# paroj/aruco

Measured on AMD Instinct MI355X. Metric: frames/sec at 1920×1080, higher is better.
Workload: dtype u8

## Files before the change

aruco_amd/capi.py:

```python
import ctypes as C
import os
import sys

import numpy as np

from .build import library_path

OK, E_INVALID, E_CAPACITY, E_UNSUPPORTED, E_HIP, E_OVERFLOW, E_BOARD_CONFIG = range(7)
THRES_FIXED, THRES_ADPT, THRES_CANNY = 0, 1, 2
CORNER_NONE, CORNER_HARRIS, CORNER_SUBPIX, CORNER_LINES = 0, 1, 2, 3
BOARD_NONE, BOARD_PIX, BOARD_METERS = -1, 0, 1

_ERR_NAMES = {1: "ARUCOHIP_E_INVALID", 2: "ARUCOHIP_E_CAPACITY", 3: "ARUCOHIP_E_UNSUPPORTED", 4: "ARUCOHIP_E_HIP",
              5: "ARUCOHIP_E_OVERFLOW", 6: "ARUCOHIP_E_BOARD_CONFIG"}


class ArucoHipError(RuntimeError):
    def __init__(self, code, msg=""):
        super().__init__("%s (%d): %s" % (_ERR_NAMES.get(code, "error"), code, msg))
        self.code = code


class Params(C.Structure):
    _fields_ = [("thres_method", C.c_int32), ("thres_param1_range", C.c_int32), ("thres_param1", C.c_double),
# ... 23 lines not shown
assert MARKER_DTYPE.itemsize == 96 and C.sizeof(Marker) == 96

SYMBOLS = [
    "arucohip_version", "arucohip_default_params", "arucohip_default_limits", "arucohip_create", "arucohip_create_ex",
    "arucohip_destroy", "arucohip_set_params", "arucohip_get_params", "arucohip_last_error_string", "arucohip_set_stream",
    "arucohip_get_stream", "arucohip_synchronize", "arucohip_detect", "arucohip_detect_batch", "arucohip_batch_status", "arucohip_batch_chunks",
    "arucohip_get_thresholded", "arucohip_get_candidates", "arucohip_threshold", "arucohip_detect_rectangles",
    "arucohip_warp", "arucohip_debug_num_contours", "arucohip_debug_contour", "arucohip_debug_candidates", "arucohip_debug_otsu",
    "arucohip_board_detect", "arucohip_calculate_extrinsics", "arucohip_stage_times", "arucohip_stage_name",
    "arucohip_enable_timing", "arucohip_kernel_times", "arucohip_threshold_exec_ms", "arucohip_kernel_name",
    "arucohip_debug_counters", "arucohip_board_detect_batch",
    "arucohip_gl_modelview", "arucohip_ogre_pose", "arucohip_gl_projection", "arucohip_ogre_projection",
    "arucohip_detect_bgr", "arucohip_detect_batch_bgr", "arucohip_bgr_to_gray", "arucohip_set_dictionary",
    "arucohip_set_decoder_callback",
    "arucohip_undistort", "arucohip_gl_modelview_n", "arucohip_gl_modelview_batch",
    "arucohip_set_pipeline_depth", "arucohip_detect_batch_submit", "arucohip_detect_batch_wait",
    "arucohip_mgpu_device_count", "arucohip_mgpu_create", "arucohip_mgpu_destroy", "arucohip_mgpu_size", "arucohip_mgpu_handle",
    "arucohip_mgpu_set_params", "arucohip_mgpu_last_error_string", "arucohip_mgpu_detect_batch", "arucohip_mgpu_detect_streams",
    "arucohip_mgpu_set_depth", "arucohip_mgpu_submit_batch", "arucohip_mgpu_submit_streams", "arucohip_mgpu_wait",
    "arucohip_compact_bytes", "arucohip_compact_markers", "arucohip_wait_event", "arucohip_detect_batch_retry_overflowed",
    "arucohip_refine_candidate_lines", "arucohip_mgpu_gather_mode", "arucohip_build_info",
]

_lib = None


def load():
    global _lib
    if _lib is not None:
        return _lib
    path = os.environ.get("ARUCOHIP_LIB") or library_path()
# ... 306 lines not shown

    def submit_host(self, frames, out, n, K=None, dist=None, marker_size=-1.0, y_perp=False):
        nf, h, w = frames.shape
        Ka, da = _f32(K), _f32(dist)
        t = C.c_int(-1)
        self._chk(self.L.arucohip_detect_batch_submit(self.h, _ptr(frames), nf, w, h, w, w * h, 0, _ptr(Ka), _ptr(da), 0 if da is None else da.size,
                                                      float(marker_size), int(bool(y_perp)), _ptr(out), out.shape[1], _ptr(n), 0, C.byref(t)))
        return t.value

    def wait(self, ticket, allow=()):
        return self._chk(self.L.arucohip_detect_batch_wait(self.h, int(ticket)), allow)

    def batch_status(self):
        return self._chk(self.L.arucohip_batch_status(self.h))

    def batch_chunks(self):
        per = C.c_int(0)
        n = self.L.arucohip_batch_chunks(self.h, C.byref(per))
        return n, per.value

    def thresholded(self, frame=0, shape=None):
        out = np.empty(shape, np.uint8)
        self._chk(self.L.arucohip_get_thresholded(self.h, frame, _ptr(out)))
        return out

    def candidates(self, frame=0, cap=512):
        q = np.zeros((cap, 4, 2), np.float32)
        n = C.c_int(0)
        self._chk(self.L.arucohip_get_candidates(self.h, frame, _ptr(q), cap, C.byref(n)))
        return q[:n.value].copy()
# ... 224 lines not shown
```

aruco_amd/csrc/capi.hip:

```cpp
#include <hip/hip_runtime.h>

#include <algorithm>
#include <cmath>
#include <cstdio>
#include <cstring>
#include <string>
#include <vector>

#include "bits_tiles.h"
#include "internal.h"

namespace ah {
void launch_rotate_x(hipStream_t s, double* rt);
}

namespace ah {
Tuning read_tuning() {
    Tuning t;
    auto geti = [](const char* name, int dflt) {
        const char* e = getenv(name);
        return (e && *e) ? atoi(e) : dflt;
    };
    t.walk_fork = geti("ARUCOHIP_WALK_FORK", 1) != 0;
    t.chain = geti("ARUCOHIP_CHAIN", 0) != 0;
    t.cand_sparse = geti("ARUCOHIP_CAND_SPARSE", 1) != 0;
    t.cand_waves = std::max(1, geti("ARUCOHIP_CAND_WAVES", 32));
    t.cand_chunks = std::max(1, geti("ARUCOHIP_CAND_CHUNKS", 16));
    t.leash = geti("ARUCOHIP_LEASH", 0);
    t.fork_after = geti("ARUCOHIP_FORK_AFTER", 3);
    t.quad_blocks = std::max(1, geti("ARUCOHIP_QUAD_BLOCKS", 12));
    t.quad_dual = geti("ARUCOHIP_QUAD_DUAL", 1) != 0;
    t.seg_skip = geti("ARUCOHIP_SEG_SKIP", 1) != 0;
    t.gen_xcd = geti("ARUCOHIP_GEN_XCD", 1) != 0;
    t.threshold_wide = geti("ARUCOHIP_THRESHOLD_WIDE", 1) != 0;
    t.threshold_eo = geti("ARUCOHIP_THRESHOLD_EO", 1) != 0;
#ifdef ARUCOHIP_STAGE_EXPERIMENT
    t.stop_after = geti("ARUCOHIP_STOP_AFTER", 99);
#endif
    t.thres_lazy = geti("ARUCOHIP_THRES_BYTES", 0) == 0;
// ... 41 lines not shown
            p = nullptr;
        return e;
    }

private:
    hipError_t release() {
        const hipError_t e = p ? (pinned ? hipHostFree(p) : hipFree(p)) : hipSuccess;
        p = nullptr, bytes = 0;
        return e;
    }
};

struct arucohip_handle {
    int device = 0;
    hipStream_t own_stream = nullptr, stream = nullptr;
    arucohip_params_t params;
    arucohip_limits_t lim;
    Buffers buf{};
    uint64_t alloc_epoch = 0;
    std::vector<Mem<void>> held;
    Mem<uint32_t> walk_scratch;
    Mem<uint8_t> patches;
    Mem<uint8_t> d_gray;
    Mem<uint8_t> d_bgr;
    arucohip_marker_t* wt_out = nullptr;
    int32_t* wt_n = nullptr;
    int wt_cap = 0;
    Mem<uint8_t> d_erode;
    Mem<uint64_t> d_canny;
    Mem<short2> d_umap_xy;
// ... 41 lines not shown
    int last_chunks = 1, last_per = 0;
    struct FrameGraph {
        hipGraphExec_t exec = nullptr;
        uint64_t key = 0;
        uint64_t seen = 0;
        uint64_t epoch = 0;
        bool thres_bytes = false;
        int disabled = 0;
    } fgraph;
    std::vector<arucohip_handle*> lanes;
    int next_ticket = 0;
    arucohip_handle* cur = nullptr;
    arucohip_handle* retry = nullptr;
    int retry_mult = 0;
    hipEvent_t ev_submit = nullptr;
    struct Pending {
        bool active = false;
        int ticket = -1, nframes = 0, cap = 0, out_on_device = 0;
        arucohip_marker_t* out = nullptr;
        int32_t* n_out = nullptr;
    } pend;
    std::string err;
};

static arucohip_handle* active(arucohip_handle* h) { return (h && h->cur) ? h->cur : h; }

static arucohip_handle* route(arucohip_handle* h, int frame, int* local) {
    if (h->last_chunks <= 1 || h->last_per <= 0) {
        *local = frame;
        return h;
    }
    const int c = std::min(frame / h->last_per, h->last_chunks - 1);
    *local = frame - c * h->last_per;
    return c == 0 ? h : h->kids[c - 1];
}

#define HIPCHK(h, expr)                                                                         \
    do {                                                                                        \
        hipError_t e_ = (expr);                                                                 \
        if (e_ != hipSuccess) {                                                                 \
// ... 63 lines not shown
    if (p->use_locked_corners && (p->corner_method == ARUCOHIP_CORNER_HARRIS || p->corner_method == ARUCOHIP_CORNER_SUBPIX) &&
        ((int)p->thres_param1 < 1 || (int)p->thres_param1 > 31))
        return fail(h, ARUCOHIP_E_UNSUPPORTED, "locked corners: window (thres_param1) outside 1..31");
    if (p->decoder_kind < ARUCOHIP_DECODER_FIDUCIAL_5X5 || p->decoder_kind > ARUCOHIP_DECODER_USER) return fail(h, ARUCOHIP_E_INVALID, "bad decoder kind");
    if (p->thres_param1_range < 0 || 2 * p->thres_param1_range + 1 > 16) return fail(h, ARUCOHIP_E_UNSUPPORTED, "threshold range too large");
    if (p->corner_method == ARUCOHIP_CORNER_SUBPIX && (int)p->thres_param1 > 15) return fail(h, ARUCOHIP_E_UNSUPPORTED, "SUBPIX window > 15");
    if (p->corner_method == ARUCOHIP_CORNER_SUBPIX && (int)p->thres_param1 < 1) return fail(h, ARUCOHIP_E_INVALID, "SUBPIX window < 1");
    return ARUCOHIP_OK;
}

extern "C" void arucohip_destroy(arucohip_handle* h);
static void free_all(arucohip_handle* h) {
    hipSetDevice(h->device);
    for (auto* k : h->kids) arucohip_destroy(k);
    h->kids.clear();
    for (auto* l : h->lanes) arucohip_destroy(l);
    h->lanes.clear();
    if (h->retry) arucohip_destroy(h->retry);
    h->retry = nullptr;
    if (h->fgraph.exec) hipGraphExecDestroy(h->fgraph.exec);
    h->fgraph.exec = nullptr;
    if (h->ev_submit) hipEventDestroy(h->ev_submit);
    if (h->ev_fork) hipEventDestroy(h->ev_fork);
    if (h->ev_thr) hipEventDestroy(h->ev_thr);
    if (h->ev_wfork) hipEventDestroy(h->ev_wfork);
    if (h->ev_wjoin) hipEventDestroy(h->ev_wjoin);
    if (h->side_stream) hipStreamDestroy(h->side_stream);
    for (auto& e : h->ev_join)
        if (e) hipEventDestroy(e);
    for (auto& set : h->ev)
        for (auto& e : set)
            if (e) hipEventDestroy(e);
    if (h->own_stream) hipStreamDestroy(h->own_stream);
}

static thread_local bool g_creating_child = false;

static void drop_retry(arucohip_handle* h) {
    if (h->retry) arucohip_destroy(h->retry);
    h->retry = nullptr, h->retry_mult = 0;
}

int arucohip_create_ex(const arucohip_params_t* params, int device, const arucohip_limits_t* lim, arucohip_handle** out) {
    if (!out || !lim) return ARUCOHIP_E_INVALID;
    *out = nullptr;
    if (lim->max_width < 32 || lim->max_height < 32 || lim->max_width > 16383 || lim->max_height > 16383 || lim->max_batch < 1 ||
        lim->max_thres_planes < 1 || lim->max_thres_planes > 16 || lim->candidates_per_frame > 512 || lim->markers_per_frame > 256 ||
        (long)lim->max_width * lim->max_height > (1L << 26) )
        return ARUCOHIP_E_INVALID;
    arucohip_handle* h = new arucohip_handle();
    h->device = device;
// ... 3 lines not shown
    else
        arucohip_default_params(&h->params);
    int rc = validate_params(h, &h->params);
    if (rc != ARUCOHIP_OK) {
        delete h;
        return rc;
    }
    auto bail = [&](hipError_t e) {
        fprintf(stderr, "arucohip_create: %s\n", hipGetErrorString(e));
        free_all(h);
        delete h;
        return ARUCOHIP_E_HIP;
    };
    hipError_t e;
    if ((e = hipSetDevice(device)) != hipSuccess) return bail(e);
    if ((e = hipStreamCreateWithFlags(&h->own_stream, hipStreamNonBlocking)) != hipSuccess) return bail(e);
    h->stream = h->own_stream;
    {
        const double mpx = (double)lim->max_batch * lim->max_width * lim->max_height / (128.0 * 1024 * 1024);
        int ns = 1;
        (void)mpx;
        if (const char* es = getenv("ARUCOHIP_STREAMS")) ns = std::min(8, std::max(1, atoi(es)));
        if (g_creating_child) ns = 1;
        h->is_child = g_creating_child;
        h->nsub = std::min(ns, lim->max_batch);
        h->cap_frames = (lim->max_batch + h->nsub - 1) / h->nsub;
    }
    const size_t F = h->cap_frames, P = F * lim->max_thres_planes, px = (size_t)lim->max_width * lim->max_height;
    Buffers& b = h->buf;
    b.tune = read_tuning();
    {
        const char* eg = getenv("ARUCOHIP_GRAPH");
// ... 66 lines not shown
        b.raw_cnt = b.trig_cnt + w_plane;
        b.ring_cnt = b.raw_cnt + w_plane;
    }
    ALLOC(h->d_small_f, 8192 * sizeof(float));
    ALLOC(h->d_small_d, 64 * sizeof(double));
    ALLOC(h->d_small_i, 64 * sizeof(int));
    ALLOC(h->d_patch, 128 * 128);
#undef ALLOC
    if ((e = hold(h, h->h_markers, (F * b.cap_markers + 1) * sizeof(arucohip_marker_t), true)) != hipSuccess) return bail(e);
    if ((e = hold(h, h->h_n, F * sizeof(int32_t), true)) != hipSuccess) return bail(e);
    if ((e = hold(h, h->h_counters, (CNT_FIXED + F) * sizeof(uint32_t), true)) != hipSuccess) return bail(e);
    for (auto& set : h->ev)
        for (auto& ev : set)
            if ((e = hipEventCreate(&ev)) != hipSuccess) return bail(e);
    if ((e = hipEventCreateWithFlags(&h->ev_thr, hipEventDisableTiming)) != hipSuccess) return bail(e);
    if ((e = hipStreamCreateWithFlags(&h->side_stream, hipStreamNonBlocking)) != hipSuccess) return bail(e);
    if ((e = hipEventCreateWithFlags(&h->ev_wfork, hipEventDisableTiming)) != hipSuccess) return bail(e);
    if ((e = hipEventCreateWithFlags(&h->ev_wjoin, hipEventDisableTiming)) != hipSuccess) return bail(e);
    if (h->nsub > 1) {
        if ((e = hipEventCreateWithFlags(&h->ev_fork, hipEventDisableTiming)) != hipSuccess) return bail(e);
        for (int i = 0; i < h->nsub - 1; i++) {
            if ((e = hipEventCreateWithFlags(&h->ev_join[i], hipEventDisableTiming)) != hipSuccess) return bail(e);
            arucohip_limits_t kl = *lim;
            kl.max_batch = h->cap_frames;
            arucohip_handle* kid = nullptr;
            g_creating_child = true;
            int krc = arucohip_create_ex(&h->params, device, &kl, &kid);
            g_creating_child = false;
            if (krc != ARUCOHIP_OK) {
                free_all(h);
                delete h;
// ... 52 lines not shown

int arucohip_synchronize(arucohip_handle* h) {
    if (!h) return ARUCOHIP_E_INVALID;
    HIPCHK(h, hipSetDevice(h->device));
    HIPCHK(h, hipStreamSynchronize(h->stream));
    return ARUCOHIP_OK;
}

int arucohip_wait_event(arucohip_handle* h, void* ev) {
    if (!h || !ev) return ARUCOHIP_E_INVALID;
    HIPCHK(h, hipSetDevice(h->device));
    HIPCHK(h, hipStreamWaitEvent(h->stream, (hipEvent_t)ev, 0));
    return ARUCOHIP_OK;
}

int arucohip_enable_timing(arucohip_handle* h, int on) {
    if (!h) return ARUCOHIP_E_INVALID;
    h->timing = on == 1;
    h->tsets = 0;
    for (auto* k : h->kids) k->timing = h->timing, k->tsets = 0;
    auto arm = [&](arucohip_handle* x) {
        x->buf.thr_stamp_on = on != 0 && x->buf.thr_stamps && x->buf.thr_acc;
        if (on && x->buf.thr_acc) {
            hipSetDevice(x->device);
            (void)hipStreamSynchronize(x->stream);
            (void)hipMemset(x->buf.thr_acc, 0, 2 * sizeof(uint64_t));
        }
    };
    arm(h);
    for (auto* k : h->kids) arm(k);
    for (auto* l : h->lanes) arucohip_enable_timing(l, on);
    return ARUCOHIP_OK;
}
static void collect_times(arucohip_handle* h) {
    for (int k = 0; k < K_COUNT; k++) h->kernel_ms[k] = 0;
    hipSetDevice(h->device);
    int total = 0;
    auto add = [&](arucohip_handle* w) {
        int n = std::min(w->tsets, TSETS);
        if (n <= 0) return;
        if (hipStreamSynchronize(w->stream) != hipSuccess) return;
        for (int s = 0; s < n; s++)
            for (int k = 0; k < K_COUNT; k++) {
                float ms = 0;
                if (hipEventElapsedTime(&ms, w->ev[s][k], w->ev[s][k + 1]) == hipSuccess) h->kernel_ms[k] += ms;
            }
        total += n;
    };
    add(h);
    for (auto* k : h->kids) add(k);
    for (auto* l : h->lanes) {
        add(l);
        for (auto* k : l->kids) add(k);
    }
    if (total > 0)
        for (int k = 0; k < K_COUNT; k++) h->kernel_ms[k] /= total;
// ... 5 lines not shown
    for (int i = 0; i < STAGE_COUNT && i < cap; i++) ms[i] = 0;
    for (int k = 0; k < K_COUNT; k++)
        if (kKernelStage[k] < cap) ms[kKernelStage[k]] += h->kernel_ms[k];
    return STAGE_COUNT;
}
const char* arucohip_kernel_name(int i) { return (i >= 0 && i < K_COUNT) ? kKernelNames[i] : ""; }
int arucohip_threshold_exec_ms(arucohip_handle* h, double* total_ms, int* launches) {
    if (!h || !total_ms || !launches) return ARUCOHIP_E_INVALID;
    hipSetDevice(h->device);
    int khz = 0;
    if (hipDeviceGetAttribute(&khz, hipDeviceAttributeWallClockRate, h->device) != hipSuccess || khz <= 0) return fail(h, ARUCOHIP_E_HIP, "no wall clock rate");
    unsigned long long ticks = 0, n = 0;
    auto add = [&](arucohip_handle* w) -> int {
        if (!w->buf.thr_acc) return ARUCOHIP_OK;
        unsigned long long v[2] = {0, 0};
        HIPCHK(h, hipStreamSynchronize(w->stream));
        HIPCHK(h, hipMemcpy(v, w->buf.thr_acc, sizeof(v), hipMemcpyDeviceToHost));
        ticks += v[0], n += v[1];
        return ARUCOHIP_OK;
    };
    int rc = add(h);
    for (auto* k : h->kids) if (rc == ARUCOHIP_OK) rc = add(k);
    for (auto* l : h->lanes) {
        if (rc == ARUCOHIP_OK) rc = add(l);
        for (auto* k : l->kids) if (rc == ARUCOHIP_OK) rc = add(k);
    }
    if (rc != ARUCOHIP_OK) return rc;
    *total_ms = (double)ticks / (double)khz, *launches = (int)n;
    return ARUCOHIP_OK;
}

// ... 86 lines not shown
    if (need > 0xFFFFFFF0ull) return fail(h, ARUCOHIP_E_CAPACITY, "batch too large for 32-bit checkpoint offsets: fewer frames per batch or a smaller max size");
    HIPCHK(h, h->walk_scratch.reserve(need * sizeof(uint32_t), h->alloc_epoch));
    h->buf.walk_scratch = h->walk_scratch;
    return ARUCOHIP_OK;
}

static int batch_prologue(arucohip_handle* h, const FrameGeom& g, int nframes, const DetectParams& dp) {
    int rc;
    if ((rc = ensure_walk_scratch(h, nframes * dp.nthr, dp))) return rc;
    if ((rc = ensure_bits_geometry(h, g.width, g.height))) return rc;
    HIPCHK(h, h->patches.reserve((size_t)h->buf.cap_flat * dp.warp_size * dp.warp_size, h->alloc_epoch));
    h->buf.patches = h->patches;
    return ARUCOHIP_OK;
}

static int user_decode_stage(arucohip_handle* h, const DetectParams& dp) {
    hipStream_t s = h->stream;
    const Buffers& b = h->buf;
    const size_t npx = (size_t)dp.warp_size * dp.warp_size;
    HIPCHK(h, h->hu_list.reserve((size_t)b.cap_flat * (sizeof(uint32_t) + sizeof(int2) + sizeof(uint32_t)) + sizeof(uint32_t), h->alloc_epoch));
    uint32_t* list = h->hu_list;
    int2* dec = (int2*)(list + b.cap_flat);
    uint32_t* order = (uint32_t*)(dec + b.cap_flat);
    uint32_t* ncand_p = order + b.cap_flat;
    HIPCHK(h, hipMemcpyAsync(ncand_p, b.counters + CNT_NCAND, sizeof(uint32_t), hipMemcpyDeviceToHost, s));
    HIPCHK(h, hipStreamSynchronize(s));
    const uint32_t n = std::min(*ncand_p, b.cap_flat);
    if (!n) return ARUCOHIP_OK;
    HIPCHK(h, h->hu_patches.reserve((size_t)n * npx + npx, h->alloc_epoch));
    uint8_t* patches = h->hu_patches;
    uint8_t* scratch = patches + (size_t)n * npx;
    HIPCHK(h, hipMemcpyAsync(list, b.cand_list, n * sizeof(uint32_t), hipMemcpyDeviceToHost, s));
// ... 44 lines not shown
        h->thres_bytes = !lazy;
        return ARUCOHIP_OK;
    }
    const size_t ntiles = (size_t)nframes * dp.nthr * ((g.width + 7) / 8) * ((g.height + 7) / 8);
    HIPCHK(h, h->d_canny.reserve(2 * ntiles * sizeof(uint64_t) + 64, h->alloc_epoch));
    uint64_t* surv = h->d_canny;
    uint64_t* edge = surv + ntiles;
    if (launch_canny(s, gray_dev, g, nframes, dp.nthr, b, surv, edge, (uint32_t*)(edge + ntiles))) return fail(h, ARUCOHIP_E_HIP, "CANNY kernels failed");
    FrameGeom tg = g;
    tg.row_stride = (size_t)g.width, tg.frame_stride = (size_t)g.width * g.height;
    launch_binary_planes(s, b.thres, tg, nframes * dp.nthr, b);
    return ARUCOHIP_OK;
}

static int detect_core(arucohip_handle* h, const uint8_t* gray_dev, const FrameGeom& g, int nframes, const DetectParams& dp, const CamModel& cam) {
    hipStream_t s = h->stream;
    Buffers& b = h->buf;
    HIPCHK(h, hipMemsetAsync(h->zero_block, 0, h->zero_words * sizeof(uint32_t), s));
    hipEvent_t* ev = h->ev[h->tsets % TSETS];
    const bool tm = h->timing;
#define MARK(i) do { if (tm) (void)hipEventRecord(ev[i], s); } while (0)
    if (h->wait_thr) HIPCHK(h, hipStreamWaitEvent(s, h->wait_thr, 0));
    MARK(K_THRESHOLD);
    {
        const int rc_ = run_threshold(h, s, gray_dev, g, nframes, dp, false);
        if (rc_) return rc_;
    }
    if (h->params.erode) {
        const bool on_tiles = !h->thres_bytes;
        HIPCHK(h, h->d_erode.reserve(on_tiles ? erode_tiles_tmp_bytes(g, nframes * dp.nthr) : (size_t)nframes * dp.nthr * g.width * g.height, h->alloc_epoch));
        if (on_tiles)
            launch_erode_tiles(s, g, nframes * dp.nthr, b, h->d_erode);
        else
            launch_erode(s, g, nframes * dp.nthr, b, h->d_erode);
    }
    if (h->ev_thr) HIPCHK(h, hipEventRecord(h->ev_thr, s));
    MARK(K_FILTER);
    if (b.seg_mode) {
        launch_start_candidates(s, g, nframes * dp.nthr, b);
        MARK(K_WALKERS);
        launch_segments(s, g, nframes * dp.nthr, dp, b);
        MARK(K_WALKERS_LONG);
        MARK(K_CONTOUR_QUADS);
        launch_contour_quads(s, g, nframes, dp, b);
    } else {
        if (RUN_STAGE(b.tune, 1)) launch_start_candidates(s, g, nframes * dp.nthr, b, dp.min_contour);
        MARK(K_WALKERS);
        WalkFork fk{b.tune.walk_fork ? h->side_stream : nullptr, h->ev_wfork, h->ev_wjoin, tm ? ev[K_WALKERS_LONG] : nullptr};
        const bool forked = RUN_STAGE(b.tune, 2) ? launch_walkers(s, fk, g, nframes * dp.nthr, dp, b) : false;
        MARK(K_CONTOUR_QUADS);
        if (RUN_STAGE(b.tune, 4)) launch_contour_quads(s, g, nframes, dp, b, forked ? 1 : 0);
        if (forked) {
            HIPCHK(h, hipStreamWaitEvent(s, h->ev_wjoin, 0));
            if (RUN_STAGE(b.tune, 4)) launch_contour_quads(s, g, nframes, dp, b, 2);
        }
    }
    MARK(K_FRAME_CANDS);
    if (RUN_STAGE(b.tune, 5)) launch_frame_candidates(s, g, nframes, dp, b);
    MARK(K_DECODE);
    const bool fused_cells = dp.decoder == ARUCOHIP_DECODER_FIDUCIAL_5X5;
    if (RUN_STAGE(b.tune, 6)) launch_decode(s, gray_dev, g, nframes, dp, b, fused_cells);
    if (dp.decoder == ARUCOHIP_DECODER_USER) {
        const int rc_ = user_decode_stage(h, dp);
        if (rc_) return rc_;
    }
    MARK(K_REFINE_LINES);
    if (RUN_STAGE(b.tune, 7)) launch_refine_lines(s, g, nframes, dp, cam, b, fused_cells);
    MARK(K_REFINE_PIXELS);
    if (dp.corner_method == ARUCOHIP_CORNER_HARRIS || dp.corner_method == ARUCOHIP_CORNER_SUBPIX) {
        if (dp.locked) launch_locked_corners(s, gray_dev, g, nframes, dp, b);
        launch_refine_pixels(s, gray_dev, g, nframes, dp, b);
    }
    MARK(K_FINALIZE);
    if (RUN_STAGE(b.tune, 8)) launch_finalize(s, g, nframes, dp, cam, b, h->wt_out, h->wt_cap, h->wt_n);
    MARK(K_POSE);
    if (RUN_STAGE(b.tune, 8) && cam.has_K && cam.marker_size > 0) launch_pose(s, nframes, cam, b);
    MARK(K_COUNT);
#undef MARK
    if (tm) h->tsets++;
    HIPCHK(h, hipGetLastError());
    h->last_w = g.width, h->last_h = g.height, h->last_frames = nframes, h->last_nthr = dp.nthr;
    h->last_gray = gray_dev, h->last_geom = g;
    return ARUCOHIP_OK;
}

static int stage_frames(arucohip_handle* h, const uint8_t* frames, int nframes, int W, int H, size_t row_stride, size_t frame_stride,
                        int on_device, int channels, const uint8_t** gray_dev, FrameGeom* g) {
    g->width = W, g->height = H;
    if (channels == 3) {
        const uint8_t* bgr = frames;
        size_t rs = row_stride, fs = frame_stride;
        if (!on_device) {
            HIPCHK(h, h->d_bgr.reserve((size_t)nframes * W * H * 3, h->alloc_epoch));
            for (int f = 0; f < nframes; f++)
// ... 37 lines not shown

static int chunk_enqueue(arucohip_handle* w, const uint8_t* frames, int nframes, int W, int H, size_t row_stride, size_t frame_stride,
                         int frames_on_device, int channels, const DetectParams& dp, const CamModel& cam, arucohip_marker_t* out, int cap, int32_t* n_out,
                         int out_on_device) {
    int rc;
    const uint8_t* gray_dev;
    FrameGeom g;
    if ((rc = stage_frames(w, frames, nframes, W, H, row_stride, frame_stride, frames_on_device, channels, &gray_dev, &g))) return rc;
    if ((rc = batch_prologue(w, g, nframes, dp))) return rc;
    const bool write_through = out_on_device && !(cam.has_K && cam.marker_size > 0) && cap > 0;
    w->wt_out = write_through ? out : nullptr, w->wt_cap = write_through ? cap : 0, w->wt_n = write_through ? n_out : nullptr;
    rc = detect_core(w, gray_dev, g, nframes, dp, cam);
    w->wt_out = nullptr, w->wt_cap = 0, w->wt_n = nullptr;
    if (rc) return rc;
    if (write_through) return ARUCOHIP_OK;
    const Buffers& b = w->buf;
    const int ncopy = std::min(cap, b.cap_markers);
    if (out_on_device) {
        if (ncopy > 0)
            HIPCHK(w, hipMemcpy2DAsync(out, (size_t)cap * sizeof(arucohip_marker_t), b.markers, (size_t)b.cap_markers * sizeof(arucohip_marker_t),
                                       (size_t)ncopy * sizeof(arucohip_marker_t), nframes, hipMemcpyDeviceToDevice, w->stream));
        HIPCHK(w, hipMemcpyAsync(n_out, b.nmarkers, nframes * sizeof(int32_t), hipMemcpyDeviceToDevice, w->stream));
        return ARUCOHIP_OK;
    }
    HIPCHK(w, hipMemcpyAsync(w->h_markers, b.markers, (size_t)nframes * b.cap_markers * sizeof(arucohip_marker_t), hipMemcpyDeviceToHost, w->stream));
    HIPCHK(w, hipMemcpyAsync(w->h_n, b.nmarkers, nframes * sizeof(int32_t), hipMemcpyDeviceToHost, w->stream));
    HIPCHK(w, hipMemcpyAsync(w->h_counters, b.counters, CNT_FIXED * sizeof(uint32_t), hipMemcpyDeviceToHost, w->stream));
    return ARUCOHIP_OK;
}

static int chunk_collect_host(arucohip_handle* h, arucohip_handle* w, int nframes, arucohip_marker_t* out, int cap, int32_t* n_out) {
    int ret = check_status(h, w->h_counters[CNT_STATUS] & ~(uint32_t)ST_MARKER_OVERFLOW);
    const Buffers& b = w->buf;
    for (int f = 0; f < nframes; f++) {
        int n = w->h_n[f];
        n_out[f] = n;
        if (n > cap) {
            if (ret == ARUCOHIP_OK) ret = fail(h, ARUCOHIP_E_CAPACITY, "marker output array too small");
            n = cap;
        }
        n = std::min(n, b.cap_markers);
        if (n > 0) std::memcpy(out + (size_t)f * cap, w->h_markers + (size_t)f * b.cap_markers, (size_t)n * sizeof(arucohip_marker_t));
// ... 4 lines not shown
static int fork_workers(arucohip_handle* h, int chunks) {
    if (chunks <= 1) return ARUCOHIP_OK;
    HIPCHK(h, hipEventRecord(h->ev_fork, h->stream));
    for (int c = 1; c < chunks; c++) HIPCHK(h, hipStreamWaitEvent(h->kids[c - 1]->stream, h->ev_fork, 0));
    return ARUCOHIP_OK;
}
static int join_workers(arucohip_handle* h, int chunks) {
    for (int c = 1; c < chunks; c++) {
        HIPCHK(h, hipEventRecord(h->ev_join[c - 1], h->kids[c - 1]->stream));
        HIPCHK(h, hipStreamWaitEvent(h->stream, h->ev_join[c - 1], 0));
    }
    return ARUCOHIP_OK;
}

static int collect_batch_host(arucohip_handle* h, int nframes, arucohip_marker_t* out, int cap, int32_t* n_out) {
    HIPCHK(h, hipStreamSynchronize(h->stream));
    const int chunks = std::max(h->last_chunks, 1), per = chunks > 1 ? h->last_per : nframes;
    int ret = ARUCOHIP_OK;
    for (int c = 0; c < chunks; c++) {
        arucohip_handle* w = c == 0 ? h : h->kids[c - 1];
        const int off = c * per, cnt = std::min(per, nframes - off);
        if (cnt <= 0) break;
        int r = chunk_collect_host(h, w, cnt, out + (size_t)off * cap, cap, n_out + off);
        if (ret == ARUCOHIP_OK) ret = r;
    }
    return ret;
}

static uint64_t digest(uint64_t hsh, const void* p, size_t n) {
    const unsigned char* c = (const unsigned char*)p;
    for (size_t i = 0; i < n; i++) hsh = (hsh ^ c[i]) * 1099511628211ull;
// ... 713 lines not shown
        }
        if ((rc = solve((int)(i2.size() / 2)))) return rc;
    }
    if (y_perp) launch_rotate_x(h->stream, h->d_small_d);
    HIPCHK(h, hipMemcpyAsync(rt, h->d_small_d, sizeof(rt), hipMemcpyDeviceToHost, h->stream));
    HIPCHK(h, hipMemcpyAsync(&ok, h->d_small_i, sizeof(int), hipMemcpyDeviceToHost, h->stream));
    HIPCHK(h, hipStreamSynchronize(h->stream));
    out->has_pose = ok;
    for (int k = 0; k < 3; k++) out->rvec[k] = rt[k], out->tvec[k] = rt[3 + k];
    *prob = float(nb) / float(nboard);
    return ARUCOHIP_OK;
}

}

extern "C" {

int arucohip_set_pipeline_depth(arucohip_handle* h, int depth) {
    if (!h || depth < 0 || depth > 8) return ARUCOHIP_E_INVALID;
    for (auto* l : h->lanes)
        if (l->pend.active) return fail(h, ARUCOHIP_E_INVALID, "a submitted batch has not been waited for");
    HIPCHK(h, hipSetDevice(h->device));
    for (auto* l : h->lanes) arucohip_destroy(l);
    h->lanes.clear();
    h->cur = nullptr, h->next_ticket = 0;
    if (depth == 0) return ARUCOHIP_OK;
    if (!h->ev_submit) HIPCHK(h, hipEventCreateWithFlags(&h->ev_submit, hipEventDisableTiming));
    for (int i = 0; i < depth; i++) {
        arucohip_handle* l = nullptr;
        int rc = arucohip_create_ex(&h->params, h->device, &h->lim, &l);
        if (rc != ARUCOHIP_OK) {
            for (auto* made : h->lanes) arucohip_destroy(made);
            h->lanes.clear();
            return fail(h, rc, "creating a pipeline lane failed (no lanes kept)");
        }
        l->decoder_fn = h->decoder_fn, l->decoder_user = h->decoder_user;
        for (auto* k : l->kids) k->decoder_fn = h->decoder_fn, k->decoder_user = h->decoder_user;
        l->timing = h->timing;
        h->lanes.push_back(l);
        if (h->d_hrm && h->hrm_count > 0) {
            std::vector<uint64_t> codes(h->hrm_count);
            HIPCHK(h, hipMemcpy(codes.data(), h->d_hrm, codes.size() * sizeof(uint64_t), hipMemcpyDeviceToHost));
            if ((rc = arucohip_set_dictionary(l, h->hrm_n, h->hrm_count, codes.data(), h->hrm_tau0, h->hrm_rate))) {
                for (auto* made : h->lanes) arucohip_destroy(made);
                h->lanes.clear();
// ... 2 lines not shown
        }
    }
    return ARUCOHIP_OK;
}

int arucohip_detect_batch_submit(arucohip_handle* h, const uint8_t* frames, int nframes, int W, int H, size_t row_stride, size_t frame_stride,
                                 int frames_on_device, const float* K, const float* dist, int ndist, float marker_size, int y_perp,
                                 arucohip_marker_t* out, int cap, int32_t* n_out, int out_on_device, int* ticket) {
    if (!h || !ticket) return ARUCOHIP_E_INVALID;
    if (h->lanes.empty()) return fail(h, ARUCOHIP_E_INVALID, "arucohip_set_pipeline_depth first");
    arucohip_handle* l = h->lanes[h->next_ticket % (int)h->lanes.size()];
    if (l->pend.active) return fail(h, ARUCOHIP_E_CAPACITY, "pipeline full: wait for the oldest ticket first");
    HIPCHK(h, hipSetDevice(h->device));
    HIPCHK(h, hipEventRecord(h->ev_submit, h->stream));
    HIPCHK(h, hipStreamWaitEvent(l->stream, h->ev_submit, 0));
    int rc = detect_batch_impl(l, frames, nframes, W, H, row_stride, frame_stride, frames_on_device, 1, K, dist, ndist, marker_size, y_perp, out, cap, n_out,
                               out_on_device, true);
    if (rc) {
        h->err = l->err;
        return rc;
    }
    l->pend.active = true, l->pend.ticket = h->next_ticket, l->pend.nframes = nframes, l->pend.cap = cap, l->pend.out_on_device = out_on_device;
    l->pend.out = out, l->pend.n_out = n_out;
    *ticket = h->next_ticket++;
    return ARUCOHIP_OK;
}

int arucohip_detect_batch_retry_overflowed(arucohip_handle* h, const uint8_t* frames, int nframes, int W, int H, size_t row_stride, size_t frame_stride,
                                           int frames_on_device, const float* K, const float* dist, int ndist, float marker_size, int y_perp,
                                           arucohip_marker_t* out, int cap, int32_t* n_out, int out_on_device, int* n_retried) {
    if (!h || !frames || !n_out || (cap > 0 && !out) || cap < 0 || nframes < 1) return ARUCOHIP_E_INVALID;
    if (n_retried) *n_retried = 0;
    HIPCHK(h, hipSetDevice(h->device));
    std::vector<int32_t> n(nframes);
    if (out_on_device)
        HIPCHK(h, hipMemcpy(n.data(), n_out, (size_t)nframes * sizeof(int32_t), hipMemcpyDeviceToHost));
// ... 42 lines not shown
            HIPCHK(h, hipMemcpy(n_out + f, &got, sizeof(int32_t), hipMemcpyHostToDevice));
        } else {
            if (ncopy > 0) std::memcpy(out + (size_t)f * cap, tmp.data(), (size_t)ncopy * sizeof(arucohip_marker_t));
            n_out[f] = got;
        }
        if (n_retried) (*n_retried)++;
    }
    return ret;
}

int arucohip_detect_batch_wait(arucohip_handle* h, int ticket) {
    if (!h || h->lanes.empty() || ticket < 0) return ARUCOHIP_E_INVALID;
    arucohip_handle* l = h->lanes[ticket % (int)h->lanes.size()];
    if (!l->pend.active || l->pend.ticket != ticket) return fail(h, ARUCOHIP_E_INVALID, "no such batch in flight");
    HIPCHK(h, hipSetDevice(h->device));
    int rc = l->pend.out_on_device ? arucohip_batch_status(l) : collect_batch_host(l, l->pend.nframes, l->pend.out, l->pend.cap, l->pend.n_out);
    l->pend.active = false;
    h->cur = l;
    if (rc) h->err = l->err;
    return rc;
}

}
```

aruco_amd/csrc/internal.h:

```cpp
#pragma once
#include <hip/hip_runtime.h>
#include <stdint.h>

#include "../../include/arucohip.h"

namespace ah {

constexpr int WAVE = 64;
constexpr int TRIG_CNT_STRIDE = 32;
constexpr int TC_CDESC = 2;
constexpr int TC_POOL = 3;
constexpr int TC_STATUS = 5;
constexpr int TC_SNAP = 4;
constexpr int WALK_BLOCKS = 16;


enum Counter {
    CNT_NMARK = 0,
    CNT_UNUSED1 = 1,
    CNT_UNUSED2 = 2,
    CNT_STATUS = 3,
    CNT_NCAND = 5,
    CNT_FIXED = 8
};
// ... 62 lines not shown
    int corner_method;
    int warp_size;
    int min_contour, max_contour;
    int bx0, by0, bx1, by1;
    int subpix_win;
    int locked, locked_wsize;
    int decoder;
    int hrm_n, hrm_count;
    uint32_t hrm_correction;
    const uint64_t* hrm_codes;
};

struct Tuning {
    int walk_fork = 1;
    int chain = 0;
    int cand_sparse = 1;
    int cand_waves = 32;
    int cand_chunks = 16;
    int leash = 0;
    int gens[32] = {};
    int ngens = 0;
    int fork_after = 3;
    int gen_xcd = 1;
    int seg_skip = 1;
    int quad_dual = 1;
    int quad_blocks = 12;
    int thres_lazy = 1;
    int threshold_wide = 1;
#ifdef ARUCOHIP_STAGE_EXPERIMENT
    int stop_after = 99;
// ... 109 lines not shown
```

include/arucohip.h:

```cpp
#ifndef ARUCOHIP_H
#define ARUCOHIP_H

#include <stddef.h>
#include <stdint.h>

#ifdef __cplusplus
extern "C" {
#endif

#define ARUCOHIP_VERSION 100

enum {
    ARUCOHIP_OK = 0,
    ARUCOHIP_E_INVALID = 1,
    ARUCOHIP_E_CAPACITY = 2,
    ARUCOHIP_E_UNSUPPORTED = 3,
    ARUCOHIP_E_HIP = 4,
    ARUCOHIP_E_OVERFLOW = 5,
    ARUCOHIP_E_BOARD_CONFIG = 6
};

enum { ARUCOHIP_THRES_FIXED = 0, ARUCOHIP_THRES_ADPT = 1, ARUCOHIP_THRES_CANNY = 2 };
enum { ARUCOHIP_CORNER_NONE = 0, ARUCOHIP_CORNER_HARRIS = 1, ARUCOHIP_CORNER_SUBPIX = 2, ARUCOHIP_CORNER_LINES = 3 };
enum { ARUCOHIP_BOARD_NONE = -1, ARUCOHIP_BOARD_PIX = 0, ARUCOHIP_BOARD_METERS = 1 };
// ... 87 lines not shown
int arucohip_undistort(arucohip_handle* h, const uint8_t* src, int nframes, int width, int height, size_t row_stride, size_t frame_stride,
                       int channels, int src_on_device, const float* K, const float* dist, int ndist, uint8_t* dst, int dst_on_device);
int arucohip_batch_status(arucohip_handle* h);
int arucohip_detect_batch_retry_overflowed(arucohip_handle* h, const uint8_t* frames, int nframes, int width, int height, size_t row_stride,
                                           size_t frame_stride, int frames_on_device, const float* K, const float* dist, int ndist,
                                           float marker_size, int y_perpendicular, arucohip_marker_t* out, int cap, int32_t* n_out,
                                           int out_on_device, int* n_retried);
int arucohip_batch_chunks(arucohip_handle* h, int* frames_per_chunk);

int arucohip_set_pipeline_depth(arucohip_handle* h, int depth);
int arucohip_detect_batch_submit(arucohip_handle* h, const uint8_t* frames, int nframes, int width, int height, size_t row_stride,
                                 size_t frame_stride, int frames_on_device, const float* K, const float* dist, int ndist,
                                 float marker_size, int y_perpendicular, arucohip_marker_t* out, int cap, int32_t* n_out,
                                 int out_on_device, int* ticket);
int arucohip_detect_batch_wait(arucohip_handle* h, int ticket);

int arucohip_get_thresholded(arucohip_handle* h, int frame, uint8_t* dst);
int arucohip_get_candidates(arucohip_handle* h, int frame, float* quads, int cap, int* n);

int arucohip_threshold(arucohip_handle* h, int method, const uint8_t* gray, int width, int height, size_t row_stride,
                       double param1, double param2, uint8_t* dst);
int arucohip_detect_rectangles(arucohip_handle* h, const uint8_t* thres, int width, int height, size_t row_stride,
                               float* quads, int cap, int* n);
int arucohip_warp(arucohip_handle* h, const uint8_t* gray, int width, int height, size_t row_stride, const float quad[8],
                  int size, uint8_t* dst);

int arucohip_refine_candidate_lines(arucohip_handle* h, const int32_t* contour_xy, int npoints, float corners[8], const float* K,
                                    const float* dist, int ndist);

int arucohip_debug_num_contours(arucohip_handle* h, int frame, int* n);
// ... 72 lines not shown
```

Baseline: 363,000.

## Split pipelined lanes into shared front and back role streams on distinct queues

When pipeline depth is set, all lanes now share two role streams: a front stream for threshold/filter/walkers and a back stream for quads, decode, refine, finalize and result copies. Tail work is deferred and enqueued only after the next batch's front work is submitted, so the front of batch N+1 overlaps the back of batch N on separate hardware queues, which a probe kernel checks. This adds event handoffs, deferred closures and extra synchronisation paths, and it risks ordering bugs between lanes.

```diff
diff --git a/aruco_amd/capi.py b/aruco_amd/capi.py
--- a/aruco_amd/capi.py
+++ b/aruco_amd/capi.py
@@ -61,7 +61,7 @@
     "arucohip_detect_bgr", "arucohip_detect_batch_bgr", "arucohip_bgr_to_gray", "arucohip_set_dictionary",
     "arucohip_set_decoder_callback",
     "arucohip_undistort", "arucohip_gl_modelview_n", "arucohip_gl_modelview_batch",
-    "arucohip_set_pipeline_depth", "arucohip_detect_batch_submit", "arucohip_detect_batch_wait",
+    "arucohip_set_pipeline_depth", "arucohip_detect_batch_submit", "arucohip_detect_batch_wait", "arucohip_debug_pipeline_queues",
     "arucohip_mgpu_device_count", "arucohip_mgpu_create", "arucohip_mgpu_destroy", "arucohip_mgpu_size", "arucohip_mgpu_handle",
     "arucohip_mgpu_set_params", "arucohip_mgpu_last_error_string", "arucohip_mgpu_detect_batch", "arucohip_mgpu_detect_streams",
     "arucohip_mgpu_set_depth", "arucohip_mgpu_submit_batch", "arucohip_mgpu_submit_streams", "arucohip_mgpu_wait",
@@ -398,6 +398,11 @@
     def batch_status(self):
         return self._chk(self.L.arucohip_batch_status(self.h))
 
+    def pipeline_queues(self):
+        q = (C.c_uint64 * 2)()
+        self._chk(self.L.arucohip_debug_pipeline_queues(self.h, q))
+        return int(q[0]), int(q[1])
+
     def batch_chunks(self):
         per = C.c_int(0)
         n = self.L.arucohip_batch_chunks(self.h, C.byref(per))
diff --git a/aruco_amd/csrc/capi.hip b/aruco_amd/csrc/capi.hip
--- a/aruco_amd/csrc/capi.hip
+++ b/aruco_amd/csrc/capi.hip
@@ -4,6 +4,7 @@
 #include <cmath>
 #include <cstdio>
 #include <cstring>
+#include <functional>
 #include <string>
 #include <vector>
 
@@ -23,6 +24,7 @@
     };
     t.walk_fork = geti("ARUCOHIP_WALK_FORK", 1) != 0;
     t.chain = geti("ARUCOHIP_CHAIN", 0) != 0;
+    t.lane_streams = geti("ARUCOHIP_LANE_STREAMS", 0) != 0;
     t.cand_sparse = geti("ARUCOHIP_CAND_SPARSE", 1) != 0;
     t.cand_waves = std::max(1, geti("ARUCOHIP_CAND_WAVES", 32));
     t.cand_chunks = std::max(1, geti("ARUCOHIP_CAND_CHUNKS", 16));
@@ -94,6 +96,7 @@
 struct arucohip_handle {
     int device = 0;
     hipStream_t own_stream = nullptr, stream = nullptr;
+    hipStream_t tail = nullptr;
     arucohip_params_t params;
     arucohip_limits_t lim;
     Buffers buf{};
@@ -165,16 +168,42 @@
     arucohip_handle* retry = nullptr;
     int retry_mult = 0;
     hipEvent_t ev_submit = nullptr;
+    hipStream_t pipe_front = nullptr, pipe_back = nullptr;
+    uint64_t pipe_queue[2] = {};
+    hipEvent_t ev_head = nullptr;
+    hipEvent_t ev_done = nullptr;
+    bool defer_tail = false;
+    std::function<int()> tail_fn;
+    arucohip_handle* deferred = nullptr;
     struct Pending {
         bool active = false;
         int ticket = -1, nframes = 0, cap = 0, out_on_device = 0;
+        int rc = 0;
         arucohip_marker_t* out = nullptr;
         int32_t* n_out = nullptr;
     } pend;
     std::string err;
 };
 
-static arucohip_handle* active(arucohip_handle* h) { return (h && h->cur) ? h->cur : h; }
+static void flush_tail(arucohip_handle* h) {
+    arucohip_handle* l = h->deferred;
+    if (!l) return;
+    h->deferred = nullptr;
+    const std::function<int()> f = std::move(l->tail_fn);
+    l->tail_fn = nullptr;
+    const int rc = f();
+    if (rc && !l->pend.rc) l->pend.rc = rc;
+}
+
+static arucohip_handle* active(arucohip_handle* h) {
+    if (!h || !h->cur) return h;
+    if (h->cur->tail) {
+        if (h->deferred == h->cur) flush_tail(h);
+        (void)hipSetDevice(h->device);
+        (void)hipEventSynchronize(h->cur->ev_done);
+    }
+    return h->cur;
+}
 
 static arucohip_handle* route(arucohip_handle* h, int frame, int* local) {
     if (h->last_chunks <= 1 || h->last_per <= 0) {
@@ -268,6 +297,11 @@
     hipSetDevice(h->device);
     for (auto* k : h->kids) arucohip_destroy(k);
     h->kids.clear();
+    if (h->pipe_front) {
+        flush_tail(h);
+        (void)hipStreamSynchronize(h->pipe_front);
+        (void)hipStreamSynchronize(h->pipe_back);
+    }
     for (auto* l : h->lanes) arucohip_destroy(l);
     h->lanes.clear();
     if (h->retry) arucohip_destroy(h->retry);
@@ -275,6 +309,8 @@
     if (h->fgraph.exec) hipGraphExecDestroy(h->fgraph.exec);
     h->fgraph.exec = nullptr;
     if (h->ev_submit) hipEventDestroy(h->ev_submit);
+    if (h->ev_head) hipEventDestroy(h->ev_head);
+    if (h->ev_done) hipEventDestroy(h->ev_done);
     if (h->ev_fork) hipEventDestroy(h->ev_fork);
     if (h->ev_thr) hipEventDestroy(h->ev_thr);
     if (h->ev_wfork) hipEventDestroy(h->ev_wfork);
@@ -286,9 +322,12 @@
         for (auto& e : set)
             if (e) hipEventDestroy(e);
     if (h->own_stream) hipStreamDestroy(h->own_stream);
+    if (h->pipe_front) hipStreamDestroy(h->pipe_front);
+    if (h->pipe_back) hipStreamDestroy(h->pipe_back);
 }
 
 static thread_local bool g_creating_child = false;
+static thread_local hipStream_t g_lane_roles[2] = {nullptr, nullptr};
 
 static void drop_retry(arucohip_handle* h) {
     if (h->retry) arucohip_destroy(h->retry);
@@ -322,8 +361,14 @@
     };
     hipError_t e;
     if ((e = hipSetDevice(device)) != hipSuccess) return bail(e);
-    if ((e = hipStreamCreateWithFlags(&h->own_stream, hipStreamNonBlocking)) != hipSuccess) return bail(e);
-    h->stream = h->own_stream;
+    if (g_lane_roles[0]) {
+        h->stream = g_lane_roles[0], h->tail = g_lane_roles[1];
+        if ((e = hipEventCreateWithFlags(&h->ev_head, hipEventDisableTiming)) != hipSuccess) return bail(e);
+        if ((e = hipEventCreateWithFlags(&h->ev_done, hipEventDisableTiming)) != hipSuccess) return bail(e);
+    } else {
+        if ((e = hipStreamCreateWithFlags(&h->own_stream, hipStreamNonBlocking)) != hipSuccess) return bail(e);
+        h->stream = h->own_stream;
+    }
     {
         const double mpx = (double)lim->max_batch * lim->max_width * lim->max_height / (128.0 * 1024 * 1024);
         int ns = 1;
@@ -420,7 +465,7 @@
         for (auto& ev : set)
             if ((e = hipEventCreate(&ev)) != hipSuccess) return bail(e);
     if ((e = hipEventCreateWithFlags(&h->ev_thr, hipEventDisableTiming)) != hipSuccess) return bail(e);
-    if ((e = hipStreamCreateWithFlags(&h->side_stream, hipStreamNonBlocking)) != hipSuccess) return bail(e);
+    if (!h->tail && (e = hipStreamCreateWithFlags(&h->side_stream, hipStreamNonBlocking)) != hipSuccess) return bail(e);
     if ((e = hipEventCreateWithFlags(&h->ev_wfork, hipEventDisableTiming)) != hipSuccess) return bail(e);
     if ((e = hipEventCreateWithFlags(&h->ev_wjoin, hipEventDisableTiming)) != hipSuccess) return bail(e);
     if (h->nsub > 1) {
@@ -503,6 +548,12 @@
     return ARUCOHIP_OK;
 }
 
+static hipError_t sync_streams(arucohip_handle* h) {
+    hipError_t e = hipStreamSynchronize(h->stream);
+    if (e == hipSuccess && h->tail) e = hipStreamSynchronize(h->tail);
+    return e;
+}
+
 int arucohip_enable_timing(arucohip_handle* h, int on) {
     if (!h) return ARUCOHIP_E_INVALID;
     h->timing = on == 1;
@@ -512,7 +563,7 @@
         x->buf.thr_stamp_on = on != 0 && x->buf.thr_stamps && x->buf.thr_acc;
         if (on && x->buf.thr_acc) {
             hipSetDevice(x->device);
-            (void)hipStreamSynchronize(x->stream);
+            (void)sync_streams(x);
             (void)hipMemset(x->buf.thr_acc, 0, 2 * sizeof(uint64_t));
         }
     };
@@ -528,7 +579,7 @@
     auto add = [&](arucohip_handle* w) {
         int n = std::min(w->tsets, TSETS);
         if (n <= 0) return;
-        if (hipStreamSynchronize(w->stream) != hipSuccess) return;
+        if (sync_streams(w) != hipSuccess) return;
         for (int s = 0; s < n; s++)
             for (int k = 0; k < K_COUNT; k++) {
                 float ms = 0;
@@ -564,7 +615,7 @@
     auto add = [&](arucohip_handle* w) -> int {
         if (!w->buf.thr_acc) return ARUCOHIP_OK;
         unsigned long long v[2] = {0, 0};
-        HIPCHK(h, hipStreamSynchronize(w->stream));
+        HIPCHK(h, sync_streams(w));
         HIPCHK(h, hipMemcpy(v, w->buf.thr_acc, sizeof(v), hipMemcpyDeviceToHost));
         ticks += v[0], n += v[1];
         return ARUCOHIP_OK;
@@ -681,8 +732,7 @@
     return ARUCOHIP_OK;
 }
 
-static int user_decode_stage(arucohip_handle* h, const DetectParams& dp) {
-    hipStream_t s = h->stream;
+static int user_decode_stage(arucohip_handle* h, hipStream_t s, const DetectParams& dp) {
     const Buffers& b = h->buf;
     const size_t npx = (size_t)dp.warp_size * dp.warp_size;
     HIPCHK(h, h->hu_list.reserve((size_t)b.cap_flat * (sizeof(uint32_t) + sizeof(int2) + sizeof(uint32_t)) + sizeof(uint32_t), h->alloc_epoch));
@@ -757,14 +807,14 @@
 }
 
 static int detect_core(arucohip_handle* h, const uint8_t* gray_dev, const FrameGeom& g, int nframes, const DetectParams& dp, const CamModel& cam) {
-    hipStream_t s = h->stream;
+    hipStream_t s = h->stream, t = h->tail ? h->tail : s;
     Buffers& b = h->buf;
     HIPCHK(h, hipMemsetAsync(h->zero_block, 0, h->zero_words * sizeof(uint32_t), s));
     hipEvent_t* ev = h->ev[h->tsets % TSETS];
     const bool tm = h->timing;
-#define MARK(i) do { if (tm) (void)hipEventRecord(ev[i], s); } while (0)
+#define MARK(i, st) do { if (tm) (void)hipEventRecord(ev[i], st); } while (0)
     if (h->wait_thr) HIPCHK(h, hipStreamWaitEvent(s, h->wait_thr, 0));
-    MARK(K_THRESHOLD);
+    MARK(K_THRESHOLD, s);
     {
         const int rc_ = run_threshold(h, s, gray_dev, g, nframes, dp, false);
         if (rc_) return rc_;
@@ -778,49 +828,67 @@
             launch_erode(s, g, nframes * dp.nthr, b, h->d_erode);
     }
     if (h->ev_thr) HIPCHK(h, hipEventRecord(h->ev_thr, s));
-    MARK(K_FILTER);
+    MARK(K_FILTER, s);
+    bool forked = false;
     if (b.seg_mode) {
         launch_start_candidates(s, g, nframes * dp.nthr, b);
-        MARK(K_WALKERS);
+        MARK(K_WALKERS, s);
         launch_segments(s, g, nframes * dp.nthr, dp, b);
-        MARK(K_WALKERS_LONG);
-        MARK(K_CONTOUR_QUADS);
+        MARK(K_WALKERS_LONG, s);
+        MARK(K_CONTOUR_QUADS, s);
         launch_contour_quads(s, g, nframes, dp, b);
     } else {
         if (RUN_STAGE(b.tune, 1)) launch_start_candidates(s, g, nframes * dp.nthr, b, dp.min_contour);
-        MARK(K_WALKERS);
-        WalkFork fk{b.tune.walk_fork ? h->side_stream : nullptr, h->ev_wfork, h->ev_wjoin, tm ? ev[K_WALKERS_LONG] : nullptr};
-        const bool forked = RUN_STAGE(b.tune, 2) ? launch_walkers(s, fk, g, nframes * dp.nthr, dp, b) : false;
-        MARK(K_CONTOUR_QUADS);
-        if (RUN_STAGE(b.tune, 4)) launch_contour_quads(s, g, nframes, dp, b, forked ? 1 : 0);
-        if (forked) {
-            HIPCHK(h, hipStreamWaitEvent(s, h->ev_wjoin, 0));
-            if (RUN_STAGE(b.tune, 4)) launch_contour_quads(s, g, nframes, dp, b, 2);
-        }
-    }
-    MARK(K_FRAME_CANDS);
-    if (RUN_STAGE(b.tune, 5)) launch_frame_candidates(s, g, nframes, dp, b);
-    MARK(K_DECODE);
-    const bool fused_cells = dp.decoder == ARUCOHIP_DECODER_FIDUCIAL_5X5;
-    if (RUN_STAGE(b.tune, 6)) launch_decode(s, gray_dev, g, nframes, dp, b, fused_cells);
-    if (dp.decoder == ARUCOHIP_DECODER_USER) {
-        const int rc_ = user_decode_stage(h, dp);
-        if (rc_) return rc_;
-    }
-    MARK(K_REFINE_LINES);
-    if (RUN_STAGE(b.tune, 7)) launch_refine_lines(s, g, nframes, dp, cam, b, fused_cells);
-    MARK(K_REFINE_PIXELS);
-    if (dp.corner_method == ARUCOHIP_CORNER_HARRIS || dp.corner_method == ARUCOHIP_CORNER_SUBPIX) {
-        if (dp.locked) launch_locked_corners(s, gray_dev, g, nframes, dp, b);
-        launch_refine_pixels(s, gray_dev, g, nframes, dp, b);
-    }
-    MARK(K_FINALIZE);
-    if (RUN_STAGE(b.tune, 8)) launch_finalize(s, g, nframes, dp, cam, b, h->wt_out, h->wt_cap, h->wt_n);
-    MARK(K_POSE);
-    if (RUN_STAGE(b.tune, 8) && cam.has_K && cam.marker_size > 0) launch_pose(s, nframes, cam, b);
-    MARK(K_COUNT);
+        MARK(K_WALKERS, s);
+        WalkFork fk{b.tune.walk_fork ? (t == s ? h->side_stream : s) : nullptr, h->ev_wfork, h->ev_wjoin, tm ? ev[K_WALKERS_LONG] : nullptr};
+        forked = RUN_STAGE(b.tune, 2) ? launch_walkers(s, fk, g, nframes * dp.nthr, dp, b) : false;
+    }
+    hipEvent_t handoff = nullptr;
+    if (t != s) {
+        handoff = forked ? h->ev_wfork : h->ev_head;
+        if (!forked) HIPCHK(h, hipEventRecord(h->ev_head, s));
+    }
+    auto back = [h, t, handoff, forked, gray_dev, g, nframes, dp, cam, ev, tm, wt_out = h->wt_out, wt_cap = h->wt_cap, wt_n = h->wt_n]() -> int {
+        const Buffers& b = h->buf;
+        if (handoff) HIPCHK(h, hipStreamWaitEvent(t, handoff, 0));
+        if (!b.seg_mode) {
+            MARK(K_CONTOUR_QUADS, t);
+            if (RUN_STAGE(b.tune, 4)) launch_contour_quads(t, g, nframes, dp, b, forked ? 1 : 0);
+            if (forked) {
+                HIPCHK(h, hipStreamWaitEvent(t, h->ev_wjoin, 0));
+                if (RUN_STAGE(b.tune, 4)) launch_contour_quads(t, g, nframes, dp, b, 2);
+            }
+        }
+        MARK(K_FRAME_CANDS, t);
+        if (RUN_STAGE(b.tune, 5)) launch_frame_candidates(t, g, nframes, dp, b);
+        MARK(K_DECODE, t);
+        const bool fused_cells = dp.decoder == ARUCOHIP_DECODER_FIDUCIAL_5X5;
+        if (RUN_STAGE(b.tune, 6)) launch_decode(t, gray_dev, g, nframes, dp, b, fused_cells);
+        if (dp.decoder == ARUCOHIP_DECODER_USER) {
+            const int rc_ = user_decode_stage(h, t, dp);
+            if (rc_) return rc_;
+        }
+        MARK(K_REFINE_LINES, t);
+        if (RUN_STAGE(b.tune, 7)) launch_refine_lines(t, g, nframes, dp, cam, b, fused_cells);
+        MARK(K_REFINE_PIXELS, t);
+        if (dp.corner_method == ARUCOHIP_CORNER_HARRIS || dp.corner_method == ARUCOHIP_CORNER_SUBPIX) {
+            if (dp.locked) launch_locked_corners(t, gray_dev, g, nframes, dp, b);
+            launch_refine_pixels(t, gray_dev, g, nframes, dp, b);
+        }
+        MARK(K_FINALIZE, t);
+        if (RUN_STAGE(b.tune, 8)) launch_finalize(t, g, nframes, dp, cam, b, wt_out, wt_cap, wt_n);
+        MARK(K_POSE, t);
+        if (RUN_STAGE(b.tune, 8) && cam.has_K && cam.marker_size > 0) launch_pose(t, nframes, cam, b);
+        MARK(K_COUNT, t);
+        HIPCHK(h, hipGetLastError());
+        return ARUCOHIP_OK;
+    };
 #undef MARK
     if (tm) h->tsets++;
+    if (h->defer_tail)
+        h->tail_fn = back;
+    else if (const int rc_ = back())
+        return rc_;
     HIPCHK(h, hipGetLastError());
     h->last_w = g.width, h->last_h = g.height, h->last_frames = nframes, h->last_nthr = dp.nthr;
     h->last_gray = gray_dev, h->last_geom = g;
@@ -888,18 +956,27 @@
     w->wt_out = nullptr, w->wt_cap = 0, w->wt_n = nullptr;
     if (rc) return rc;
     if (write_through) return ARUCOHIP_OK;
-    const Buffers& b = w->buf;
-    const int ncopy = std::min(cap, b.cap_markers);
-    if (out_on_device) {
-        if (ncopy > 0)
-            HIPCHK(w, hipMemcpy2DAsync(out, (size_t)cap * sizeof(arucohip_marker_t), b.markers, (size_t)b.cap_markers * sizeof(arucohip_marker_t),
-                                       (size_t)ncopy * sizeof(arucohip_marker_t), nframes, hipMemcpyDeviceToDevice, w->stream));
-        HIPCHK(w, hipMemcpyAsync(n_out, b.nmarkers, nframes * sizeof(int32_t), hipMemcpyDeviceToDevice, w->stream));
+    auto results = [w, nframes, out, cap, n_out, out_on_device]() -> int {
+        const Buffers& b = w->buf;
+        hipStream_t t = w->tail ? w->tail : w->stream;
+        const int ncopy = std::min(cap, b.cap_markers);
+        if (out_on_device) {
+            if (ncopy > 0)
+                HIPCHK(w, hipMemcpy2DAsync(out, (size_t)cap * sizeof(arucohip_marker_t), b.markers, (size_t)b.cap_markers * sizeof(arucohip_marker_t),
+                                           (size_t)ncopy * sizeof(arucohip_marker_t), nframes, hipMemcpyDeviceToDevice, t));
+            HIPCHK(w, hipMemcpyAsync(n_out, b.nmarkers, nframes * sizeof(int32_t), hipMemcpyDeviceToDevice, t));
+            return ARUCOHIP_OK;
+        }
+        HIPCHK(w, hipMemcpyAsync(w->h_markers, b.markers, (size_t)nframes * b.cap_markers * sizeof(arucohip_marker_t), hipMemcpyDeviceToHost, t));
+        HIPCHK(w, hipMemcpyAsync(w->h_n, b.nmarkers, nframes * sizeof(int32_t), hipMemcpyDeviceToHost, t));
+        HIPCHK(w, hipMemcpyAsync(w->h_counters, b.counters, CNT_FIXED * sizeof(uint32_t), hipMemcpyDeviceToHost, t));
         return ARUCOHIP_OK;
-    }
-    HIPCHK(w, hipMemcpyAsync(w->h_markers, b.markers, (size_t)nframes * b.cap_markers * sizeof(arucohip_marker_t), hipMemcpyDeviceToHost, w->stream));
-    HIPCHK(w, hipMemcpyAsync(w->h_n, b.nmarkers, nframes * sizeof(int32_t), hipMemcpyDeviceToHost, w->stream));
-    HIPCHK(w, hipMemcpyAsync(w->h_counters, b.counters, CNT_FIXED * sizeof(uint32_t), hipMemcpyDeviceToHost, w->stream));
+    };
+    if (!w->defer_tail) return results();
+    w->tail_fn = [core = std::move(w->tail_fn), results]() {
+        const int r = core();
+        return r ? r : results();
+    };
     return ARUCOHIP_OK;
 }
 
@@ -934,7 +1011,7 @@
 }
 
 static int collect_batch_host(arucohip_handle* h, int nframes, arucohip_marker_t* out, int cap, int32_t* n_out) {
-    HIPCHK(h, hipStreamSynchronize(h->stream));
+    HIPCHK(h, h->tail ? hipEventSynchronize(h->ev_done) : hipStreamSynchronize(h->stream));
     const int chunks = std::max(h->last_chunks, 1), per = chunks > 1 ? h->last_per : nframes;
     int ret = ARUCOHIP_OK;
     for (int c = 0; c < chunks; c++) {
@@ -1678,21 +1755,73 @@
 
 }
 
+__global__ void queue_probe_kernel(unsigned long long* out) {
+    if (threadIdx.x == 0) *out = (unsigned long long)(uintptr_t)__builtin_amdgcn_queue_ptr();
+}
+
+static int queue_of(arucohip_handle* h, hipStream_t st, uint64_t* q) {
+    unsigned long long* d = (unsigned long long*)h->d_small_d;
+    hipLaunchKernelGGL(queue_probe_kernel, dim3(1), dim3(64), 0, st, d);
+    HIPCHK(h, hipGetLastError());
+    HIPCHK(h, hipStreamSynchronize(st));
+    HIPCHK(h, hipMemcpy(q, d, sizeof(*q), hipMemcpyDeviceToHost));
+    return ARUCOHIP_OK;
+}
+
+static int make_role_streams(arucohip_handle* h) {
+    if (h->pipe_front) return ARUCOHIP_OK;
+    HIPCHK(h, hipStreamCreateWithFlags(&h->pipe_front, hipStreamNonBlocking));
+    HIPCHK(h, hipStreamCreateWithFlags(&h->pipe_back, hipStreamNonBlocking));
+    int rc;
+    if ((rc = queue_of(h, h->pipe_front, &h->pipe_queue[0])) || (rc = queue_of(h, h->pipe_back, &h->pipe_queue[1]))) return rc;
+    if (h->pipe_queue[0] == h->pipe_queue[1]) {
+        hipStream_t other = nullptr;
+        uint64_t q = 0;
+        HIPCHK(h, hipStreamCreateWithFlags(&other, hipStreamNonBlocking));
+        if ((rc = queue_of(h, other, &q))) {
+            (void)hipStreamDestroy(other);
+            return rc;
+        }
+        if (q != h->pipe_queue[0]) std::swap(h->pipe_back, other), h->pipe_queue[1] = q;
+        HIPCHK(h, hipStreamDestroy(other));
+    }
+    return ARUCOHIP_OK;
+}
+
 extern "C" {
+
+int arucohip_debug_pipeline_queues(arucohip_handle* h, uint64_t* queues) {
+    if (!h || !queues) return ARUCOHIP_E_INVALID;
+    if (!h->pipe_front || h->lanes.empty() || !h->lanes[0]->tail) return fail(h, ARUCOHIP_E_INVALID, "the pipeline lanes do not run on the role streams");
+    queues[0] = h->pipe_queue[0], queues[1] = h->pipe_queue[1];
+    return ARUCOHIP_OK;
+}
 
 int arucohip_set_pipeline_depth(arucohip_handle* h, int depth) {
     if (!h || depth < 0 || depth > 8) return ARUCOHIP_E_INVALID;
     for (auto* l : h->lanes)
         if (l->pend.active) return fail(h, ARUCOHIP_E_INVALID, "a submitted batch has not been waited for");
     HIPCHK(h, hipSetDevice(h->device));
+    if (h->pipe_front) {
+        flush_tail(h);
+        HIPCHK(h, hipStreamSynchronize(h->pipe_front));
+        HIPCHK(h, hipStreamSynchronize(h->pipe_back));
+    }
     for (auto* l : h->lanes) arucohip_destroy(l);
     h->lanes.clear();
     h->cur = nullptr, h->next_ticket = 0;
     if (depth == 0) return ARUCOHIP_OK;
     if (!h->ev_submit) HIPCHK(h, hipEventCreateWithFlags(&h->ev_submit, hipEventDisableTiming));
+    const bool roles = h->nsub == 1 && !h->buf.tune.lane_streams;
+    if (roles) {
+        const int rc = make_role_streams(h);
+        if (rc) return rc;
+    }
     for (int i = 0; i < depth; i++) {
         arucohip_handle* l = nullptr;
+        if (roles) g_lane_roles[0] = h->pipe_front, g_lane_roles[1] = h->pipe_back;
         int rc = arucohip_create_ex(&h->params, h->device, &h->lim, &l);
+        g_lane_roles[0] = g_lane_roles[1] = nullptr;
         if (rc != ARUCOHIP_OK) {
             for (auto* made : h->lanes) arucohip_destroy(made);
             h->lanes.clear();
@@ -1725,12 +1854,28 @@
     HIPCHK(h, hipSetDevice(h->device));
     HIPCHK(h, hipEventRecord(h->ev_submit, h->stream));
     HIPCHK(h, hipStreamWaitEvent(l->stream, h->ev_submit, 0));
+    if (l->tail) HIPCHK(h, hipStreamWaitEvent(l->stream, l->ev_done, 0));
+    l->defer_tail = l->tail != nullptr;
     int rc = detect_batch_impl(l, frames, nframes, W, H, row_stride, frame_stride, frames_on_device, 1, K, dist, ndist, marker_size, y_perp, out, cap, n_out,
                                out_on_device, true);
+    l->defer_tail = false;
+    if (rc == ARUCOHIP_OK && l->tail) {
+        l->tail_fn = [l, inner = std::move(l->tail_fn), out_on_device]() -> int {
+            if (const int r = inner()) return r;
+            if (out_on_device)
+                HIPCHK(l, hipMemcpyAsync(l->h_counters, l->buf.counters, CNT_FIXED * sizeof(uint32_t), hipMemcpyDeviceToHost, l->tail));
+            HIPCHK(l, hipEventRecord(l->ev_done, l->tail));
+            return ARUCOHIP_OK;
+        };
+    }
     if (rc) {
+        l->tail_fn = nullptr;
         h->err = l->err;
         return rc;
     }
+    flush_tail(h);
+    if (l->tail) h->deferred = l;
+    l->pend.rc = 0;
     l->pend.active = true, l->pend.ticket = h->next_ticket, l->pend.nframes = nframes, l->pend.cap = cap, l->pend.out_on_device = out_on_device;
     l->pend.out = out, l->pend.n_out = n_out;
     *ticket = h->next_ticket++;
@@ -1803,7 +1948,18 @@
     arucohip_handle* l = h->lanes[ticket % (int)h->lanes.size()];
     if (!l->pend.active || l->pend.ticket != ticket) return fail(h, ARUCOHIP_E_INVALID, "no such batch in flight");
     HIPCHK(h, hipSetDevice(h->device));
-    int rc = l->pend.out_on_device ? arucohip_batch_status(l) : collect_batch_host(l, l->pend.nframes, l->pend.out, l->pend.cap, l->pend.n_out);
+    flush_tail(h);
+    int rc;
+    if (l->pend.rc) {
+        rc = l->pend.rc;
+        l->pend.rc = 0;
+    } else if (!l->pend.out_on_device)
+        rc = collect_batch_host(l, l->pend.nframes, l->pend.out, l->pend.cap, l->pend.n_out);
+    else if (l->tail) {
+        HIPCHK(h, hipEventSynchronize(l->ev_done));
+        rc = check_status(l, l->h_counters[CNT_STATUS]);
+    } else
+        rc = arucohip_batch_status(l);
     l->pend.active = false;
     h->cur = l;
     if (rc) h->err = l->err;
diff --git a/aruco_amd/csrc/internal.h b/aruco_amd/csrc/internal.h
--- a/aruco_amd/csrc/internal.h
+++ b/aruco_amd/csrc/internal.h
@@ -100,6 +100,7 @@
 struct Tuning {
     int walk_fork = 1;
     int chain = 0;
+    int lane_streams = 0;
     int cand_sparse = 1;
     int cand_waves = 32;
     int cand_chunks = 16;
diff --git a/include/arucohip.h b/include/arucohip.h
--- a/include/arucohip.h
+++ b/include/arucohip.h
@@ -125,6 +125,7 @@
                                  float marker_size, int y_perpendicular, arucohip_marker_t* out, int cap, int32_t* n_out,
                                  int out_on_device, int* ticket);
 int arucohip_detect_batch_wait(arucohip_handle* h, int ticket);
+int arucohip_debug_pipeline_queues(arucohip_handle* h, uint64_t* queues);
 
 int arucohip_get_thresholded(arucohip_handle* h, int frame, uint8_t* dst);
 int arucohip_get_candidates(arucohip_handle* h, int frame, float* quads, int cap, int* n);
```

Measured after the change: 387,800 (median of 6 runs). +6.8%, better.
